# xlite-dev/LeetCUDA

Measured on AMD Instinct MI355X. Metric: achieved fp16 TFLOPS vs MI355X MFMA peak: HGEMM 8192^3; FA-2 fwd S=4096 D=128, higher is better.
Workload: dtype f16 (fp32 MFMA accumulate)

## Files before the change

### leetcuda_amd/csrc/hgemm_w4y.hip

```cpp
#pragma once
#include "hgemm_w4x.hip"

namespace lc {

struct W4yNNSrc {
  const char* ub;
  unsigned b_off[2];
  unsigned bq, bkt;
};
LC_DEVINL void w4y_nn_src_init(W4yNNSrc& s, const half_t* B, int n0, int N, int wave, int lane) {
  const int pp = lane & 15, kr = lane >> 4;
#pragma unroll
  for (int par = 0; par < 2; ++par) {
    const int pair = (pp >> 1) ^ ((kr << 1) | par);
    s.b_off[par] = (unsigned)kr * (unsigned)N * 2u + (unsigned)((pair * 2 + (pp & 1)) * 16);
  }
  s.ub = (const char*)(B + (size_t)(wave * 16) * N + n0);
  s.bq = (unsigned)N * 8u;
  s.bkt = (unsigned)N * 128u;
}

template <bool ALPHA = false>
LC_DEVINL void w4y_epilogue_b2(char* slot, half_t* C, int N, int m0, int n0, int wave, int wr, int wc, int lane, float alpha = 1.f) {
  asm volatile("" : "+v"(lane));
// ... 158 lines not shown
    const u32x4_t w4y_rb = {(uint32_t)__builtin_amdgcn_readfirstlane((uint32_t)pb),
                            (uint32_t)__builtin_amdgcn_readfirstlane((uint32_t)(pb >> 32)) & 0xffffu, 0x7fffffffu, 0x00020000u};
    const uint32_t w4y_a0 = __builtin_amdgcn_readfirstlane(lds_addr32(smem));
    const uint32_t w4y_wv = (uint32_t)wave * 1024u;
    const uint32_t w4y_blk = __builtin_amdgcn_readfirstlane((uint32_t)src.a_blk);
    const uint32_t w4y_ao0 = src.a_off[0], w4y_ao1 = src.a_off[1];
    uint32_t w4y_t, w4y_acur, w4y_anxt, w4y_b0, w4y_b1, w4y_b2, w4y_soff, w4y_t2off, w4y_tmp, w4y_swp;
    if constexpr (B_KN) {
      const uint32_t w4y_wvb = (uint32_t)wave * 4096u;
      const uint32_t w4y_bq = __builtin_amdgcn_readfirstlane(nsrc.bq), w4y_bkt = __builtin_amdgcn_readfirstlane(nsrc.bkt);
      const uint32_t w4y_bo0 = nsrc.b_off[0], w4y_bo1 = nsrc.b_off[1];
      const int ti = lane & 15, tg = lane >> 4;
      const uint32_t w4y_bk = (uint32_t)(wc * HALF_BYTES + (8 * tg + (ti >> 2)) * 256 + (ti & 3) * 8);
      const uint32_t w4y_key = (uint32_t)(((ti >> 2) << 1) | (tg & 1));
      uint32_t w4y_t2offb;
#include "hgemm_w4y_loop_nn.inc"
    } else if constexpr (SCHED == 0) {
#include "hgemm_w4y_loop0.inc"
    } else if constexpr (SCHED == 1) {
#include "hgemm_w4y_loop1.inc"
#ifdef LC_DIAG
    } else if constexpr (SCHED == 3) {
#include "hgemm_w4y_loop3.inc"
    } else if constexpr (SCHED == 4) {
#include "hgemm_w4y_loop4.inc"
    } else if constexpr (SCHED == 5) {
#include "hgemm_w4y_loop5.inc"
    } else if constexpr (SCHED == 6) {
#include "hgemm_w4y_loop2.inc"
#endif
    } else {
// ... 22 lines not shown
```

### leetcuda_amd/csrc/tu_plan.hip

```cpp
#include <stdio.h>
#include <string.h>

#include <algorithm>

#include "lc_plan.h"

namespace lc {

#define LC_KNOB(name, dflt, valid, diag) tune_t g_tune_##name{dflt};
#include "lc_knobs.inc"

Knobs read_knobs() {
  Knobs k;
#define LC_KNOB(name, dflt, valid, diag)
#define LC_KNOB_SNAP(name, dflt, valid, diag) k.name = g_tune_##name;
#include "lc_knobs.inc"
  return k;
}

namespace {
bool ok_attn_nw(int v) {
  return v == 0 || v == 512 || v == 513 || v == 514 || v == 515 || v == 517 || v == 8 || v == 4 || v == 2;
}
bool ok_01(int v) { return v == 0 || v == 1; }
// ... 263 lines not shown
  if (knob == 0 || T <= ncu || R == 0 || !(knob == 3 ? 4 * R <= 3 * ncu : knob == 4 || 2 * R <= ncu)) return t;
  t.nblk = T - R;
  if (mid_ok && knob != 2) {
    t.tmw = tile_knob == 1 ? 1 : tile_knob == 2 ? 2 : (8 * R <= ncu ? 1 : 2);
    t.ns = (t.tmw == 1 ? 8 : 4) * R <= ncu ? 3 : 2;
  }
  return t;
}

}

int plan_hgemm(const Knobs& k, int M, int N, int K, bool b_kn, int variant, bool al, HgemmPlan* out) {
  HgemmPlan p{};
  p.k = k;
  p.variant = variant;
  p.sched = b_kn ? 1 : k.w4y_sched;
  p.tail = TailSplit{-1, 0, 0, 0};
  const bool k64 = K % BK == 0, k32 = K % 32 == 0 && K >= BK;
  const bool tiles256 = (M % BM == 0) && (N % BN == 0) && k64 && al;
  const bool tiles128 = (M % BM1 == 0) && (N % BN1 == 0) && k32 && al;
  const bool edge_ok = al && K % 8 == 0 && (!b_kn || N % 8 == 0);
  const bool w4y_ok = tiles128 && M >= BM && N >= BN && w4_effective_variant(LC_HGEMM_MFMA256W4Y, b_kn, N, K) == LC_HGEMM_MFMA256W4Y;
  if (variant == LC_HGEMM_AUTO) {
    const long wg256 = (long)(M / BM) * (N / BN), rcu = rule_cus(k);
    const bool tiles64 = (M % 64 == 0) && (N % 64 == 0) && k32 && al;
    p.mid = mid_tile_auto(k, M, N, K, b_kn, true);
    if (2 * wg256 > rcu && (tiles256 || (k.hgemm_auto == LC_HGEMM_MFMA256W4Y && w4y_ok))) {
      p.fam = wg256 < rcu && p.mid.tmw > 0 && p.mid.wgs > wg256 ? HFam::MID : HFam::TILE256;
      p.variant = k.hgemm_auto;
    } else {
      p.rag = tiles128 ? RaggedPlan{0, 0, 0, 0, 0, 0, 1} : ragged_plan(k, M, N, K, al, b_kn, true);
// ... 380 lines not shown
```

### leetcuda_amd/csrc/tu_w4.hip

```cpp
#include "lc_launch.h"
#include "hgemm_w4y.hip"

namespace lc {
namespace {
template <bool B_KN, bool BUF, int DG>
int launch_w4_one(const half_t* A, const half_t* B, half_t* C, int M, int N, int K, int tiles_m, int tiles_n, int pw,
                  hipStream_t st) {
  auto kern = hgemm_w4b_kernel<B_KN, BUF, DG>;
  if (int rc = set_dyn_lds(kern, W4B_LDS)) return rc;
  hipLaunchKernelGGL(kern, dim3(tiles_m * tiles_n), dim3(256), W4B_LDS, st, A, B, C, M, N, K, tiles_m, tiles_n, pw);
  return check_launch();
}

template <bool B_KN, int Y>
int launch_w4x_one(const half_t* A, const half_t* B, half_t* C, int M, int N, int K, int tiles_m, int tiles_n, int pw,
                   int nblk_arg, hipStream_t st) {
  auto kern = [] {
    if constexpr (Y < 0) return hgemm_w4x_kernel<B_KN>;
    else return hgemm_w4y_kernel<B_KN, Y>;
  }();
  if (int rc = set_dyn_lds(kern, W4B_LDS)) return rc;
  const int nblk = nblk_arg > 0 ? nblk_arg : tiles_m * tiles_n;
  if constexpr (Y < 0) {
    hipLaunchKernelGGL(kern, dim3(nblk), dim3(256), W4B_LDS, st, A, B, C, M, N, K, tiles_m, tiles_n, pw);
// ... 23 lines not shown
#endif
  if constexpr (!B_KN) {
    if (variant == LC_HGEMM_MFMA256W4X) return launch_w4x_one<B_KN, -1>(A, B, C, M, N, K, tiles_m, tiles_n, pw, nblk, st);
    if (variant == LC_HGEMM_MFMA256W4Y) {
      if (sched == 0) return launch_w4x_one<B_KN, 0>(A, B, C, M, N, K, tiles_m, tiles_n, pw, nblk, st);
      if (sched == 1) return launch_w4x_one<B_KN, 1>(A, B, C, M, N, K, tiles_m, tiles_n, pw, nblk, st);
#ifdef LC_DIAG
      if (sched == 3) return launch_w4x_one<B_KN, 3>(A, B, C, M, N, K, tiles_m, tiles_n, pw, nblk, st);
      if (sched == 4) return launch_w4x_one<B_KN, 4>(A, B, C, M, N, K, tiles_m, tiles_n, pw, nblk, st);
      if (sched == 5) return launch_w4x_one<B_KN, 5>(A, B, C, M, N, K, tiles_m, tiles_n, pw, nblk, st);
      if (sched == 6) return launch_w4x_one<B_KN, 6>(A, B, C, M, N, K, tiles_m, tiles_n, pw, nblk, st);
#endif
      return launch_w4x_one<B_KN, 2>(A, B, C, M, N, K, tiles_m, tiles_n, pw, nblk, st);
    }
  } else {
    if (variant == LC_HGEMM_MFMA256W4Y) return launch_w4x_one<B_KN, 1>(A, B, C, M, N, K, tiles_m, tiles_n, pw, nblk, st);
  }
  if (variant == LC_HGEMM_MFMA256W4C || variant == LC_HGEMM_MFMA256W4X || variant == LC_HGEMM_MFMA256W4Y)
    return launch_w4_one<B_KN, true, 0>(A, B, C, M, N, K, tiles_m, tiles_n, pw, st);
  return launch_w4_one<B_KN, false, 0>(A, B, C, M, N, K, tiles_m, tiles_n, pw, st);
}
}

int launch_w4_family(const half_t* A, const half_t* B, half_t* C, int M, int N, int K, int variant, int sched, int stamps, int abl, bool b_kn,
                     int tiles_m, int tiles_n, int panel_w, int nblk, hipStream_t st) {
  return b_kn ? launch_w4_t<true>(A, B, C, M, N, K, variant, sched, stamps, abl, tiles_m, tiles_n, panel_w, nblk, st)
              : launch_w4_t<false>(A, B, C, M, N, K, variant, sched, stamps, abl, tiles_m, tiles_n, panel_w, nblk, st);
}
}
```

Before: 1500.

## Add paired double-buffered B-fragment loop for NN (B_KN) W4Y HGEMM path

Adds a new hand-scheduled inline-asm main loop for the B_KN (row-major B) W4Y kernel. It double-buffers the transposed B register fragments (ds_read_b64_tr_b16 into alternating v128-191 / v192-255 banks) so the next iteration's B reads interleave with the current iteration's MFMAs, and the loop is unrolled in pairs. The old NN loop stays reachable only under LC_DIAG with sched 6. It uses nearly the whole VGPR file and depends on the exact order of waitcnts and barriers, so it raises register pressure and the risk of scheduling hazards.

```diff
diff --git a/leetcuda_amd/csrc/hgemm_w4y.hip b/leetcuda_amd/csrc/hgemm_w4y.hip
--- a/leetcuda_amd/csrc/hgemm_w4y.hip
+++ b/leetcuda_amd/csrc/hgemm_w4y.hip
@@ -196,7 +196,14 @@
       const uint32_t w4y_bk = (uint32_t)(wc * HALF_BYTES + (8 * tg + (ti >> 2)) * 256 + (ti & 3) * 8);
       const uint32_t w4y_key = (uint32_t)(((ti >> 2) << 1) | (tg & 1));
       uint32_t w4y_t2offb;
+#ifdef LC_DIAG
+      if constexpr (SCHED == 6) {
 #include "hgemm_w4y_loop_nn.inc"
+      } else
+#endif
+      {
+#include "hgemm_w4y_loop_nn_pair.inc"
+      }
     } else if constexpr (SCHED == 0) {
 #include "hgemm_w4y_loop0.inc"
     } else if constexpr (SCHED == 1) {
diff --git a/leetcuda_amd/csrc/hgemm_w4y_loop_nn_pair.inc b/leetcuda_amd/csrc/hgemm_w4y_loop_nn_pair.inc
--- /dev/null
+++ b/leetcuda_amd/csrc/hgemm_w4y_loop_nn_pair.inc
@@ -0,0 +1,610 @@
+asm volatile(
+    "s_mov_b32 %[t], 0\n\t"
+    "s_mov_b32 %[acur], %[a0]\n\t"
+    "s_add_u32 %[anxt], %[a0], 0x8000\n\t"
+    "s_add_u32 %[b0], %[a0], 0x10000\n\t"
+    "s_add_u32 %[b1], %[a0], 0x18000\n\t"
+    "s_add_u32 %[b2], %[a0], 0x20000\n\t"
+    "v_xor_b32_e32 v56, 0, %[key]\n\t"
+    "v_xor_b32_e32 v57, 1, %[key]\n\t"
+    "v_xor_b32_e32 v58, 2, %[key]\n\t"
+    "v_xor_b32_e32 v59, 3, %[key]\n\t"
+    "v_xor_b32_e32 v60, 4, %[key]\n\t"
+    "v_xor_b32_e32 v61, 5, %[key]\n\t"
+    "v_xor_b32_e32 v62, 6, %[key]\n\t"
+    "v_xor_b32_e32 v63, 7, %[key]\n\t"
+    "v_lshl_add_u32 v56, v56, 5, %[bk]\n\t"
+    "v_lshl_add_u32 v57, v57, 5, %[bk]\n\t"
+    "v_lshl_add_u32 v58, v58, 5, %[bk]\n\t"
+    "v_lshl_add_u32 v59, v59, 5, %[bk]\n\t"
+    "v_lshl_add_u32 v60, v60, 5, %[bk]\n\t"
+    "v_lshl_add_u32 v61, v61, 5, %[bk]\n\t"
+    "v_lshl_add_u32 v62, v62, 5, %[bk]\n\t"
+    "v_lshl_add_u32 v63, v63, 5, %[bk]\n\t"
+    "v_add_u32_e32 v56, %[b0], v56\n\t"
+    "v_add_u32_e32 v57, %[b0], v57\n\t"
+    "v_add_u32_e32 v58, %[b0], v58\n\t"
+    "v_add_u32_e32 v59, %[b0], v59\n\t"
+    "v_add_u32_e32 v60, %[b0], v60\n\t"
+    "v_add_u32_e32 v61, %[b0], v61\n\t"
+    "v_add_u32_e32 v62, %[b0], v62\n\t"
+    "v_add_u32_e32 v63, %[b0], v63\n\t"
+    "v_add_u32_e32 v54, %[acur], %[ar0]\n\t"
+    "v_add_u32_e32 v55, %[acur], %[ar1]\n\t"
+    "ds_read_b128 v[64:67], v54 offset:0\n\t"
+    "ds_read_b128 v[96:99], v55 offset:0\n\t"
+    "ds_read_b64_tr_b16 v[128:129], v56 offset:0\n\t"
+    "ds_read_b64_tr_b16 v[130:131], v56 offset:1024\n\t"
+    "ds_read_b64_tr_b16 v[160:161], v56 offset:8192\n\t"
+    "ds_read_b64_tr_b16 v[162:163], v56 offset:9216\n\t"
+    "ds_read_b64_tr_b16 v[132:133], v57 offset:0\n\t"
+    "ds_read_b64_tr_b16 v[134:135], v57 offset:1024\n\t"
+    "ds_read_b64_tr_b16 v[164:165], v57 offset:8192\n\t"
+    "ds_read_b64_tr_b16 v[166:167], v57 offset:9216\n\t"
+    "ds_read_b64_tr_b16 v[136:137], v58 offset:0\n\t"
+    "ds_read_b64_tr_b16 v[138:139], v58 offset:1024\n\t"
+    "ds_read_b64_tr_b16 v[168:169], v58 offset:8192\n\t"
+    "ds_read_b64_tr_b16 v[170:171], v58 offset:9216\n\t"
+    "ds_read_b64_tr_b16 v[140:141], v59 offset:0\n\t"
+    "ds_read_b64_tr_b16 v[142:143], v59 offset:1024\n\t"
+    "ds_read_b64_tr_b16 v[172:173], v59 offset:8192\n\t"
+    "ds_read_b64_tr_b16 v[174:175], v59 offset:9216\n\t"
+    "ds_read_b64_tr_b16 v[144:145], v60 offset:0\n\t"
+    "ds_read_b64_tr_b16 v[146:147], v60 offset:1024\n\t"
+    "ds_read_b64_tr_b16 v[176:177], v60 offset:8192\n\t"
+    "ds_read_b64_tr_b16 v[178:179], v60 offset:9216\n\t"
+    "ds_read_b64_tr_b16 v[148:149], v61 offset:0\n\t"
+    "ds_read_b64_tr_b16 v[150:151], v61 offset:1024\n\t"
+    "ds_read_b64_tr_b16 v[180:181], v61 offset:8192\n\t"
+    "ds_read_b64_tr_b16 v[182:183], v61 offset:9216\n\t"
+    "ds_read_b64_tr_b16 v[152:153], v62 offset:0\n\t"
+    "ds_read_b64_tr_b16 v[154:155], v62 offset:1024\n\t"
+    "ds_read_b64_tr_b16 v[184:185], v62 offset:8192\n\t"
+    "ds_read_b64_tr_b16 v[186:187], v62 offset:9216\n\t"
+    "ds_read_b64_tr_b16 v[156:157], v63 offset:0\n\t"
+    "ds_read_b64_tr_b16 v[158:159], v63 offset:1024\n\t"
+    "ds_read_b64_tr_b16 v[188:189], v63 offset:8192\n\t"
+    "ds_read_b64_tr_b16 v[190:191], v63 offset:9216\n\t"
+    "s_sub_u32 %[swp], %[kt], 1\n\t"
+    "s_min_u32 %[swp], %[swp], 2\n\t"
+    "s_add_u32 %[swp], %[swp], %[stg]\n\t"
+    "s_cmp_ge_u32 %[swp], %[kt]\n\t"
+    "s_cselect_b32 %[t2off], %[kt], 0\n\t"
+    "s_sub_u32 %[swp], %[swp], %[t2off]\n\t"
+    "s_lshl_b32 %[t2off], %[swp], 7\n\t"
+    "s_mul_i32 %[t2offb], %[swp], %[bkt]\n\t"
+    ".Lw4y_loop_%=:\n\t"
+    "s_waitcnt lgkmcnt(0)\n\t"
+    "v_mfma_f32_16x16x32_f16 a[0:3], v[128:131], v[64:67], a[0:3]\n\t"
+    "v_mfma_f32_16x16x32_f16 a[0:3], v[160:163], v[96:99], a[0:3]\n\t"
+    "ds_read_b128 v[68:71], v54 offset:2048\n\t"
+    "v_mfma_f32_16x16x32_f16 a[4:7], v[132:135], v[64:67], a[4:7]\n\t"
+    "s_add_u32 %[tmp], %[b2], %[wvb]\n\t"
+    "v_mfma_f32_16x16x32_f16 a[4:7], v[164:167], v[96:99], a[4:7]\n\t"
+    "s_add_u32 m0, %[tmp], 0\n\t"
+    "s_mov_b32 %[soff], %[t2offb]\n\t"
+    "v_mfma_f32_16x16x32_f16 a[8:11], v[136:139], v[64:67], a[8:11]\n\t"
+    "buffer_load_dwordx4 %[bo0], %[rb], %[soff] offen lds\n\t"
+    "v_mfma_f32_16x16x32_f16 a[8:11], v[168:171], v[96:99], a[8:11]\n\t"
+    "ds_read_b128 v[100:103], v55 offset:2048\n\t"
+    "v_mfma_f32_16x16x32_f16 a[12:15], v[140:143], v[64:67], a[12:15]\n\t"
+    "v_mfma_f32_16x16x32_f16 a[12:15], v[172:175], v[96:99], a[12:15]\n\t"
+    "v_mfma_f32_16x16x32_f16 a[16:19], v[144:147], v[64:67], a[16:19]\n\t"
+    "v_mfma_f32_16x16x32_f16 a[16:19], v[176:179], v[96:99], a[16:19]\n\t"
+    "ds_read_b128 v[72:75], v54 offset:4096\n\t"
+    "v_mfma_f32_16x16x32_f16 a[20:23], v[148:151], v[64:67], a[20:23]\n\t"
+    "v_mfma_f32_16x16x32_f16 a[20:23], v[180:183], v[96:99], a[20:23]\n\t"
+    "s_add_u32 m0, %[tmp], 1024\n\t"
+    "s_add_u32 %[soff], %[soff], %[bq]\n\t"
+    "v_mfma_f32_16x16x32_f16 a[24:27], v[152:155], v[64:67], a[24:27]\n\t"
+    "buffer_load_dwordx4 %[bo0], %[rb], %[soff] offen lds\n\t"
+    "v_mfma_f32_16x16x32_f16 a[24:27], v[184:187], v[96:99], a[24:27]\n\t"
+    "ds_read_b128 v[104:107], v55 offset:4096\n\t"
+    "v_mfma_f32_16x16x32_f16 a[28:31], v[156:159], v[64:67], a[28:31]\n\t"
+    "v_mfma_f32_16x16x32_f16 a[28:31], v[188:191], v[96:99], a[28:31]\n\t"
+    "s_waitcnt lgkmcnt(2)\n\t"
+    "v_mfma_f32_16x16x32_f16 a[32:35], v[128:131], v[68:71], a[32:35]\n\t"
+    "v_mfma_f32_16x16x32_f16 a[32:35], v[160:163], v[100:103], a[32:35]\n\t"
+    "ds_read_b128 v[76:79], v54 offset:6144\n\t"
+    "v_mfma_f32_16x16x32_f16 a[36:39], v[132:135], v[68:71], a[36:39]\n\t"
+    "v_mfma_f32_16x16x32_f16 a[36:39], v[164:167], v[100:103], a[36:39]\n\t"
+    "s_add_u32 m0, %[tmp], 2048\n\t"
+    "s_add_u32 %[soff], %[soff], %[bq]\n\t"
+    "v_mfma_f32_16x16x32_f16 a[40:43], v[136:139], v[68:71], a[40:43]\n\t"
+    "buffer_load_dwordx4 %[bo1], %[rb], %[soff] offen lds\n\t"
+    "v_mfma_f32_16x16x32_f16 a[40:43], v[168:171], v[100:103], a[40:43]\n\t"
+    "ds_read_b128 v[108:111], v55 offset:6144\n\t"
+    "v_mfma_f32_16x16x32_f16 a[44:47], v[140:143], v[68:71], a[44:47]\n\t"
+    "v_mfma_f32_16x16x32_f16 a[44:47], v[172:175], v[100:103], a[44:47]\n\t"
+    "v_mfma_f32_16x16x32_f16 a[48:51], v[144:147], v[68:71], a[48:51]\n\t"
+    "v_mfma_f32_16x16x32_f16 a[48:51], v[176:179], v[100:103], a[48:51]\n\t"
+    "ds_read_b128 v[80:83], v54 offset:8192\n\t"
+    "v_mfma_f32_16x16x32_f16 a[52:55], v[148:151], v[68:71], a[52:55]\n\t"
+    "v_mfma_f32_16x16x32_f16 a[52:55], v[180:183], v[100:103], a[52:55]\n\t"
+    "s_add_u32 m0, %[tmp], 3072\n\t"
+    "s_add_u32 %[soff], %[soff], %[bq]\n\t"
+    "v_mfma_f32_16x16x32_f16 a[56:59], v[152:155], v[68:71], a[56:59]\n\t"
+    "buffer_load_dwordx4 %[bo1], %[rb], %[soff] offen lds\n\t"
+    "v_mfma_f32_16x16x32_f16 a[56:59], v[184:187], v[100:103], a[56:59]\n\t"
+    "ds_read_b128 v[112:115], v55 offset:8192\n\t"
+    "v_mfma_f32_16x16x32_f16 a[60:63], v[156:159], v[68:71], a[60:63]\n\t"
+    "v_mfma_f32_16x16x32_f16 a[60:63], v[188:191], v[100:103], a[60:63]\n\t"
+    "s_waitcnt lgkmcnt(4)\n\t"
+    "v_mfma_f32_16x16x32_f16 a[64:67], v[128:131], v[72:75], a[64:67]\n\t"
+    "v_mfma_f32_16x16x32_f16 a[64:67], v[160:163], v[104:107], a[64:67]\n\t"
+    "ds_read_b128 v[84:87], v54 offset:10240\n\t"
+    "v_mfma_f32_16x16x32_f16 a[68:71], v[132:135], v[72:75], a[68:71]\n\t"
+    "v_mfma_f32_16x16x32_f16 a[68:71], v[164:167], v[104:107], a[68:71]\n\t"
+    "s_add_u32 m0, %[tmp], 16384\n\t"
+    "s_add_u32 %[soff], %[t2offb], 256\n\t"
+    "v_mfma_f32_16x16x32_f16 a[72:75], v[136:139], v[72:75], a[72:75]\n\t"
+    "buffer_load_dwordx4 %[bo0], %[rb], %[soff] offen lds\n\t"
+    "v_mfma_f32_16x16x32_f16 a[72:75], v[168:171], v[104:107], a[72:75]\n\t"
+    "ds_read_b128 v[116:119], v55 offset:10240\n\t"
+    "v_mfma_f32_16x16x32_f16 a[76:79], v[140:143], v[72:75], a[76:79]\n\t"
+    "v_mfma_f32_16x16x32_f16 a[76:79], v[172:175], v[104:107], a[76:79]\n\t"
+    "v_mfma_f32_16x16x32_f16 a[80:83], v[144:147], v[72:75], a[80:83]\n\t"
+    "v_mfma_f32_16x16x32_f16 a[80:83], v[176:179], v[104:107], a[80:83]\n\t"
+    "ds_read_b128 v[88:91], v54 offset:12288\n\t"
+    "v_mfma_f32_16x16x32_f16 a[84:87], v[148:151], v[72:75], a[84:87]\n\t"
+    "v_mfma_f32_16x16x32_f16 a[84:87], v[180:183], v[104:107], a[84:87]\n\t"
+    "s_add_u32 m0, %[tmp], 17408\n\t"
+    "s_add_u32 %[soff], %[soff], %[bq]\n\t"
+    "v_mfma_f32_16x16x32_f16 a[88:91], v[152:155], v[72:75], a[88:91]\n\t"
+    "buffer_load_dwordx4 %[bo0], %[rb], %[soff] offen lds\n\t"
+    "v_mfma_f32_16x16x32_f16 a[88:91], v[184:187], v[104:107], a[88:91]\n\t"
+    "ds_read_b128 v[120:123], v55 offset:12288\n\t"
+    "v_mfma_f32_16x16x32_f16 a[92:95], v[156:159], v[72:75], a[92:95]\n\t"
+    "v_mfma_f32_16x16x32_f16 a[92:95], v[188:191], v[104:107], a[92:95]\n\t"
+    "s_waitcnt lgkmcnt(6)\n\t"
+    "v_mfma_f32_16x16x32_f16 a[96:99], v[128:131], v[76:79], a[96:99]\n\t"
+    "v_mfma_f32_16x16x32_f16 a[96:99], v[160:163], v[108:111], a[96:99]\n\t"
+    "ds_read_b128 v[92:95], v54 offset:14336\n\t"
+    "v_mfma_f32_16x16x32_f16 a[100:103], v[132:135], v[76:79], a[100:103]\n\t"
+    "v_mfma_f32_16x16x32_f16 a[100:103], v[164:167], v[108:111], a[100:103]\n\t"
+    "s_add_u32 m0, %[tmp], 18432\n\t"
+    "s_add_u32 %[soff], %[soff], %[bq]\n\t"
+    "v_mfma_f32_16x16x32_f16 a[104:107], v[136:139], v[76:79], a[104:107]\n\t"
+    "buffer_load_dwordx4 %[bo1], %[rb], %[soff] offen lds\n\t"
+    "v_mfma_f32_16x16x32_f16 a[104:107], v[168:171], v[108:111], a[104:107]\n\t"
+    "ds_read_b128 v[124:127], v55 offset:14336\n\t"
+    "v_mfma_f32_16x16x32_f16 a[108:111], v[140:143], v[76:79], a[108:111]\n\t"
+    "v_mfma_f32_16x16x32_f16 a[108:111], v[172:175], v[108:111], a[108:111]\n\t"
+    "v_mfma_f32_16x16x32_f16 a[112:115], v[144:147], v[76:79], a[112:115]\n\t"
+    "v_mfma_f32_16x16x32_f16 a[112:115], v[176:179], v[108:111], a[112:115]\n\t"
+    "v_mfma_f32_16x16x32_f16 a[116:119], v[148:151], v[76:79], a[116:119]\n\t"
+    "v_mfma_f32_16x16x32_f16 a[116:119], v[180:183], v[108:111], a[116:119]\n\t"
+    "s_add_u32 m0, %[tmp], 19456\n\t"
+    "s_add_u32 %[soff], %[soff], %[bq]\n\t"
+    "v_mfma_f32_16x16x32_f16 a[120:123], v[152:155], v[76:79], a[120:123]\n\t"
+    "buffer_load_dwordx4 %[bo1], %[rb], %[soff] offen lds\n\t"
+    "v_mfma_f32_16x16x32_f16 a[120:123], v[184:187], v[108:111], a[120:123]\n\t"
+    "v_mfma_f32_16x16x32_f16 a[124:127], v[156:159], v[76:79], a[124:127]\n\t"
+    "v_mfma_f32_16x16x32_f16 a[124:127], v[188:191], v[108:111], a[124:127]\n\t"
+    "s_waitcnt vmcnt(8) lgkmcnt(0)\n\t"
+    "v_mfma_f32_16x16x32_f16 a[128:131], v[128:131], v[80:83], a[128:131]\n\t"
+    "s_barrier\n\t"
+    "v_add_u32_e32 v54, %[anxt], %[ar0]\n\t"
+    "s_add_u32 %[tmp], %[acur], %[wv]\n\t"
+    "s_sub_u32 %[swp], %[b1], %[b0]\n\t"
+    "v_mfma_f32_16x16x32_f16 a[128:131], v[160:163], v[112:115], a[128:131]\n\t"
+    "v_add_u32_e32 v55, %[anxt], %[ar1]\n\t"
+    "v_add_u32_e32 v56, %[swp], v56\n\t"
+    "v_add_u32_e32 v57, %[swp], v57\n\t"
+    "v_mfma_f32_16x16x32_f16 a[132:135], v[132:135], v[80:83], a[132:135]\n\t"
+    "s_add_u32 m0, %[tmp], 0\n\t"
+    "s_mov_b32 %[soff], %[t2off]\n\t"
+    "v_add_u32_e32 v58, %[swp], v58\n\t"
+    "v_add_u32_e32 v59, %[swp], v59\n\t"
+    "v_mfma_f32_16x16x32_f16 a[132:135], v[164:167], v[112:115], a[132:135]\n\t"
+    "buffer_load_dwordx4 %[ao0], %[ra], %[soff] offen lds\n\t"
+    "v_add_u32_e32 v60, %[swp], v60\n\t"
+    "v_add_u32_e32 v61, %[swp], v61\n\t"
+    "v_mfma_f32_16x16x32_f16 a[136:139], v[136:139], v[80:83], a[136:139]\n\t"
+    "v_add_u32_e32 v62, %[swp], v62\n\t"
+    "ds_read_b128 v[64:67], v54 offset:0\n\t"
+    "v_mfma_f32_16x16x32_f16 a[136:139], v[168:171], v[112:115], a[136:139]\n\t"
+    "v_add_u32_e32 v63, %[swp], v63\n\t"
+    "ds_read_b128 v[96:99], v55 offset:0\n\t"
+    "v_mfma_f32_16x16x32_f16 a[140:143], v[140:143], v[80:83], a[140:143]\n\t"
+    "ds_read_b64_tr_b16 v[192:193], v56 offset:0\n\t"
+    "v_mfma_f32_16x16x32_f16 a[140:143], v[172:175], v[112:115], a[140:143]\n\t"
+    "ds_read_b64_tr_b16 v[194:195], v56 offset:1024\n\t"
+    "v_mfma_f32_16x16x32_f16 a[144:147], v[144:147], v[80:83], a[144:147]\n\t"
+    "s_mov_b32 %[swp], %[b0]\n\t"
+    "s_mov_b32 %[b0], %[b1]\n\t"
+    "s_mov_b32 %[b1], %[b2]\n\t"
+    "s_mov_b32 %[b2], %[swp]\n\t"
+    "s_mov_b32 %[swp], %[acur]\n\t"
+    "s_mov_b32 %[acur], %[anxt]\n\t"
+    "v_mfma_f32_16x16x32_f16 a[144:147], v[176:179], v[112:115], a[144:147]\n\t"
+    "s_add_u32 m0, %[tmp], 4096\n\t"
+    "s_add_u32 %[soff], %[soff], %[blk]\n\t"
+    "v_mfma_f32_16x16x32_f16 a[148:151], v[148:151], v[80:83], a[148:151]\n\t"
+    "buffer_load_dwordx4 %[ao1], %[ra], %[soff] offen lds\n\t"
+    "v_mfma_f32_16x16x32_f16 a[148:151], v[180:183], v[112:115], a[148:151]\n\t"
+    "ds_read_b64_tr_b16 v[224:225], v56 offset:8192\n\t"
+    "v_mfma_f32_16x16x32_f16 a[152:155], v[152:155], v[80:83], a[152:155]\n\t"
+    "ds_read_b64_tr_b16 v[226:227], v56 offset:9216\n\t"
+    "v_mfma_f32_16x16x32_f16 a[152:155], v[184:187], v[112:115], a[152:155]\n\t"
+    "ds_read_b64_tr_b16 v[196:197], v57 offset:0\n\t"
+    "v_mfma_f32_16x16x32_f16 a[156:159], v[156:159], v[80:83], a[156:159]\n\t"
+    "s_mov_b32 %[anxt], %[swp]\n\t"
+    "v_mfma_f32_16x16x32_f16 a[156:159], v[188:191], v[112:115], a[156:159]\n\t"
+    "ds_read_b64_tr_b16 v[198:199], v57 offset:1024\n\t"
+    "v_mfma_f32_16x16x32_f16 a[160:163], v[128:131], v[84:87], a[160:163]\n\t"
+    "s_add_u32 m0, %[tmp], 8192\n\t"
+    "s_add_u32 %[soff], %[soff], %[blk]\n\t"
+    "v_mfma_f32_16x16x32_f16 a[160:163], v[160:163], v[116:119], a[160:163]\n\t"
+    "buffer_load_dwordx4 %[ao0], %[ra], %[soff] offen lds\n\t"
+    "v_mfma_f32_16x16x32_f16 a[164:167], v[132:135], v[84:87], a[164:167]\n\t"
+    "ds_read_b64_tr_b16 v[228:229], v57 offset:8192\n\t"
+    "v_mfma_f32_16x16x32_f16 a[164:167], v[164:167], v[116:119], a[164:167]\n\t"
+    "ds_read_b64_tr_b16 v[230:231], v57 offset:9216\n\t"
+    "v_mfma_f32_16x16x32_f16 a[168:171], v[136:139], v[84:87], a[168:171]\n\t"
+    "ds_read_b64_tr_b16 v[200:201], v58 offset:0\n\t"
+    "v_mfma_f32_16x16x32_f16 a[168:171], v[168:171], v[116:119], a[168:171]\n\t"
+    "s_add_u32 %[swp], %[t], 3\n\t"
+    "v_mfma_f32_16x16x32_f16 a[172:175], v[140:143], v[84:87], a[172:175]\n\t"
+    "ds_read_b64_tr_b16 v[202:203], v58 offset:1024\n\t"
+    "v_mfma_f32_16x16x32_f16 a[172:175], v[172:175], v[116:119], a[172:175]\n\t"
+    "s_add_u32 m0, %[tmp], 12288\n\t"
+    "s_add_u32 %[soff], %[soff], %[blk]\n\t"
+    "v_mfma_f32_16x16x32_f16 a[176:179], v[144:147], v[84:87], a[176:179]\n\t"
+    "buffer_load_dwordx4 %[ao1], %[ra], %[soff] offen lds\n\t"
+    "v_mfma_f32_16x16x32_f16 a[176:179], v[176:179], v[116:119], a[176:179]\n\t"
+    "ds_read_b64_tr_b16 v[232:233], v58 offset:8192\n\t"
+    "v_mfma_f32_16x16x32_f16 a[180:183], v[148:151], v[84:87], a[180:183]\n\t"
+    "ds_read_b64_tr_b16 v[234:235], v58 offset:9216\n\t"
+    "v_mfma_f32_16x16x32_f16 a[180:183], v[180:183], v[116:119], a[180:183]\n\t"
+    "s_sub_u32 %[t2off], %[kt], 1\n\t"
+    "v_mfma_f32_16x16x32_f16 a[184:187], v[152:155], v[84:87], a[184:187]\n\t"
+    "ds_read_b64_tr_b16 v[204:205], v59 offset:0\n\t"
+    "v_mfma_f32_16x16x32_f16 a[184:187], v[184:187], v[116:119], a[184:187]\n\t"
+    "ds_read_b64_tr_b16 v[206:207], v59 offset:1024\n\t"
+    "v_mfma_f32_16x16x32_f16 a[188:191], v[156:159], v[84:87], a[188:191]\n\t"
+    "s_add_u32 m0, %[tmp], 16384\n\t"
+    "s_add_u32 %[soff], %[soff], %[blk]\n\t"
+    "v_mfma_f32_16x16x32_f16 a[188:191], v[188:191], v[116:119], a[188:191]\n\t"
+    "buffer_load_dwordx4 %[ao0], %[ra], %[soff] offen lds\n\t"
+    "v_mfma_f32_16x16x32_f16 a[192:195], v[128:131], v[88:91], a[192:195]\n\t"
+    "ds_read_b64_tr_b16 v[236:237], v59 offset:8192\n\t"
+    "v_mfma_f32_16x16x32_f16 a[192:195], v[160:163], v[120:123], a[192:195]\n\t"
+    "s_min_u32 %[swp], %[swp], %[t2off]\n\t"
+    "v_mfma_f32_16x16x32_f16 a[196:199], v[132:135], v[88:91], a[196:199]\n\t"
+    "ds_read_b64_tr_b16 v[238:239], v59 offset:9216\n\t"
+    "v_mfma_f32_16x16x32_f16 a[196:199], v[164:167], v[120:123], a[196:199]\n\t"
+    "ds_read_b64_tr_b16 v[208:209], v60 offset:0\n\t"
+    "v_mfma_f32_16x16x32_f16 a[200:203], v[136:139], v[88:91], a[200:203]\n\t"
+    "ds_read_b64_tr_b16 v[210:211], v60 offset:1024\n\t"
+    "v_mfma_f32_16x16x32_f16 a[200:203], v[168:171], v[120:123], a[200:203]\n\t"
+    "s_add_u32 m0, %[tmp], 20480\n\t"
+    "s_add_u32 %[soff], %[soff], %[blk]\n\t"
+    "v_mfma_f32_16x16x32_f16 a[204:207], v[140:143], v[88:91], a[204:207]\n\t"
+    "buffer_load_dwordx4 %[ao1], %[ra], %[soff] offen lds\n\t"
+    "v_mfma_f32_16x16x32_f16 a[204:207], v[172:175], v[120:123], a[204:207]\n\t"
+    "ds_read_b64_tr_b16 v[240:241], v60 offset:8192\n\t"
+    "v_mfma_f32_16x16x32_f16 a[208:211], v[144:147], v[88:91], a[208:211]\n\t"
+    "s_add_u32 %[swp], %[swp], %[stg]\n\t"
+    "v_mfma_f32_16x16x32_f16 a[208:211], v[176:179], v[120:123], a[208:211]\n\t"
+    "ds_read_b64_tr_b16 v[242:243], v60 offset:9216\n\t"
+    "v_mfma_f32_16x16x32_f16 a[212:215], v[148:151], v[88:91], a[212:215]\n\t"
+    "ds_read_b64_tr_b16 v[212:213], v61 offset:0\n\t"
+    "v_mfma_f32_16x16x32_f16 a[212:215], v[180:183], v[120:123], a[212:215]\n\t"
+    "ds_read_b64_tr_b16 v[214:215], v61 offset:1024\n\t"
+    "v_mfma_f32_16x16x32_f16 a[216:219], v[152:155], v[88:91], a[216:219]\n\t"
+    "s_add_u32 m0, %[tmp], 24576\n\t"
+    "s_add_u32 %[soff], %[soff], %[blk]\n\t"
+    "v_mfma_f32_16x16x32_f16 a[216:219], v[184:187], v[120:123], a[216:219]\n\t"
+    "buffer_load_dwordx4 %[ao0], %[ra], %[soff] offen lds\n\t"
+    "v_mfma_f32_16x16x32_f16 a[220:223], v[156:159], v[88:91], a[220:223]\n\t"
+    "s_cmp_ge_u32 %[swp], %[kt]\n\t"
+    "s_cselect_b32 %[t2off], %[kt], 0\n\t"
+    "v_mfma_f32_16x16x32_f16 a[220:223], v[188:191], v[120:123], a[220:223]\n\t"
+    "ds_read_b64_tr_b16 v[244:245], v61 offset:8192\n\t"
+    "v_mfma_f32_16x16x32_f16 a[224:227], v[128:131], v[92:95], a[224:227]\n\t"
+    "ds_read_b64_tr_b16 v[246:247], v61 offset:9216\n\t"
+    "v_mfma_f32_16x16x32_f16 a[224:227], v[160:163], v[124:127], a[224:227]\n\t"
+    "ds_read_b64_tr_b16 v[216:217], v62 offset:0\n\t"
+    "v_mfma_f32_16x16x32_f16 a[228:231], v[132:135], v[92:95], a[228:231]\n\t"
+    "ds_read_b64_tr_b16 v[218:219], v62 offset:1024\n\t"
+    "v_mfma_f32_16x16x32_f16 a[228:231], v[164:167], v[124:127], a[228:231]\n\t"
+    "s_add_u32 m0, %[tmp], 28672\n\t"
+    "s_add_u32 %[soff], %[soff], %[blk]\n\t"
+    "v_mfma_f32_16x16x32_f16 a[232:235], v[136:139], v[92:95], a[232:235]\n\t"
+    "buffer_load_dwordx4 %[ao1], %[ra], %[soff] offen lds\n\t"
+    "v_mfma_f32_16x16x32_f16 a[232:235], v[168:171], v[124:127], a[232:235]\n\t"
+    "s_sub_u32 %[swp], %[swp], %[t2off]\n\t"
+    "v_mfma_f32_16x16x32_f16 a[236:239], v[140:143], v[92:95], a[236:239]\n\t"
+    "ds_read_b64_tr_b16 v[248:249], v62 offset:8192\n\t"
+    "v_mfma_f32_16x16x32_f16 a[236:239], v[172:175], v[124:127], a[236:239]\n\t"
+    "ds_read_b64_tr_b16 v[250:251], v62 offset:9216\n\t"
+    "v_mfma_f32_16x16x32_f16 a[240:243], v[144:147], v[92:95], a[240:243]\n\t"
+    "ds_read_b64_tr_b16 v[220:221], v63 offset:0\n\t"
+    "v_mfma_f32_16x16x32_f16 a[240:243], v[176:179], v[124:127], a[240:243]\n\t"
+    "s_lshl_b32 %[t2off], %[swp], 7\n\t"
+    "v_mfma_f32_16x16x32_f16 a[244:247], v[148:151], v[92:95], a[244:247]\n\t"
+    "ds_read_b64_tr_b16 v[222:223], v63 offset:1024\n\t"
+    "v_mfma_f32_16x16x32_f16 a[244:247], v[180:183], v[124:127], a[244:247]\n\t"
+    "ds_read_b64_tr_b16 v[252:253], v63 offset:8192\n\t"
+    "v_mfma_f32_16x16x32_f16 a[248:251], v[152:155], v[92:95], a[248:251]\n\t"
+    "ds_read_b64_tr_b16 v[254:255], v63 offset:9216\n\t"
+    "v_mfma_f32_16x16x32_f16 a[248:251], v[184:187], v[124:127], a[248:251]\n\t"
+    "s_mul_i32 %[t2offb], %[swp], %[bkt]\n\t"
+    "v_mfma_f32_16x16x32_f16 a[252:255], v[156:159], v[92:95], a[252:255]\n\t"
+    "s_add_u32 %[t], %[t], 1\n\t"
+    "s_cmp_lt_u32 %[t], %[kt]\n\t"
+    "v_mfma_f32_16x16x32_f16 a[252:255], v[188:191], v[124:127], a[252:255]\n\t"
+    "s_cbranch_scc0 .Lw4y_exit_%=\n\t"
+    "s_waitcnt lgkmcnt(0)\n\t"
+    "v_mfma_f32_16x16x32_f16 a[0:3], v[192:195], v[64:67], a[0:3]\n\t"
+    "v_mfma_f32_16x16x32_f16 a[0:3], v[224:227], v[96:99], a[0:3]\n\t"
+    "ds_read_b128 v[68:71], v54 offset:2048\n\t"
+    "v_mfma_f32_16x16x32_f16 a[4:7], v[196:199], v[64:67], a[4:7]\n\t"
+    "s_add_u32 %[tmp], %[b2], %[wvb]\n\t"
+    "v_mfma_f32_16x16x32_f16 a[4:7], v[228:231], v[96:99], a[4:7]\n\t"
+    "s_add_u32 m0, %[tmp], 0\n\t"
+    "s_mov_b32 %[soff], %[t2offb]\n\t"
+    "v_mfma_f32_16x16x32_f16 a[8:11], v[200:203], v[64:67], a[8:11]\n\t"
+    "buffer_load_dwordx4 %[bo0], %[rb], %[soff] offen lds\n\t"
+    "v_mfma_f32_16x16x32_f16 a[8:11], v[232:235], v[96:99], a[8:11]\n\t"
+    "ds_read_b128 v[100:103], v55 offset:2048\n\t"
+    "v_mfma_f32_16x16x32_f16 a[12:15], v[204:207], v[64:67], a[12:15]\n\t"
+    "v_mfma_f32_16x16x32_f16 a[12:15], v[236:239], v[96:99], a[12:15]\n\t"
+    "v_mfma_f32_16x16x32_f16 a[16:19], v[208:211], v[64:67], a[16:19]\n\t"
+    "v_mfma_f32_16x16x32_f16 a[16:19], v[240:243], v[96:99], a[16:19]\n\t"
+    "ds_read_b128 v[72:75], v54 offset:4096\n\t"
+    "v_mfma_f32_16x16x32_f16 a[20:23], v[212:215], v[64:67], a[20:23]\n\t"
+    "v_mfma_f32_16x16x32_f16 a[20:23], v[244:247], v[96:99], a[20:23]\n\t"
+    "s_add_u32 m0, %[tmp], 1024\n\t"
+    "s_add_u32 %[soff], %[soff], %[bq]\n\t"
+    "v_mfma_f32_16x16x32_f16 a[24:27], v[216:219], v[64:67], a[24:27]\n\t"
+    "buffer_load_dwordx4 %[bo0], %[rb], %[soff] offen lds\n\t"
+    "v_mfma_f32_16x16x32_f16 a[24:27], v[248:251], v[96:99], a[24:27]\n\t"
+    "ds_read_b128 v[104:107], v55 offset:4096\n\t"
+    "v_mfma_f32_16x16x32_f16 a[28:31], v[220:223], v[64:67], a[28:31]\n\t"
+    "v_mfma_f32_16x16x32_f16 a[28:31], v[252:255], v[96:99], a[28:31]\n\t"
+    "s_waitcnt lgkmcnt(2)\n\t"
+    "v_mfma_f32_16x16x32_f16 a[32:35], v[192:195], v[68:71], a[32:35]\n\t"
+    "v_mfma_f32_16x16x32_f16 a[32:35], v[224:227], v[100:103], a[32:35]\n\t"
+    "ds_read_b128 v[76:79], v54 offset:6144\n\t"
+    "v_mfma_f32_16x16x32_f16 a[36:39], v[196:199], v[68:71], a[36:39]\n\t"
+    "v_mfma_f32_16x16x32_f16 a[36:39], v[228:231], v[100:103], a[36:39]\n\t"
+    "s_add_u32 m0, %[tmp], 2048\n\t"
+    "s_add_u32 %[soff], %[soff], %[bq]\n\t"
+    "v_mfma_f32_16x16x32_f16 a[40:43], v[200:203], v[68:71], a[40:43]\n\t"
+    "buffer_load_dwordx4 %[bo1], %[rb], %[soff] offen lds\n\t"
+    "v_mfma_f32_16x16x32_f16 a[40:43], v[232:235], v[100:103], a[40:43]\n\t"
+    "ds_read_b128 v[108:111], v55 offset:6144\n\t"
+    "v_mfma_f32_16x16x32_f16 a[44:47], v[204:207], v[68:71], a[44:47]\n\t"
+    "v_mfma_f32_16x16x32_f16 a[44:47], v[236:239], v[100:103], a[44:47]\n\t"
+    "v_mfma_f32_16x16x32_f16 a[48:51], v[208:211], v[68:71], a[48:51]\n\t"
+    "v_mfma_f32_16x16x32_f16 a[48:51], v[240:243], v[100:103], a[48:51]\n\t"
+    "ds_read_b128 v[80:83], v54 offset:8192\n\t"
+    "v_mfma_f32_16x16x32_f16 a[52:55], v[212:215], v[68:71], a[52:55]\n\t"
+    "v_mfma_f32_16x16x32_f16 a[52:55], v[244:247], v[100:103], a[52:55]\n\t"
+    "s_add_u32 m0, %[tmp], 3072\n\t"
+    "s_add_u32 %[soff], %[soff], %[bq]\n\t"
+    "v_mfma_f32_16x16x32_f16 a[56:59], v[216:219], v[68:71], a[56:59]\n\t"
+    "buffer_load_dwordx4 %[bo1], %[rb], %[soff] offen lds\n\t"
+    "v_mfma_f32_16x16x32_f16 a[56:59], v[248:251], v[100:103], a[56:59]\n\t"
+    "ds_read_b128 v[112:115], v55 offset:8192\n\t"
+    "v_mfma_f32_16x16x32_f16 a[60:63], v[220:223], v[68:71], a[60:63]\n\t"
+    "v_mfma_f32_16x16x32_f16 a[60:63], v[252:255], v[100:103], a[60:63]\n\t"
+    "s_waitcnt lgkmcnt(4)\n\t"
+    "v_mfma_f32_16x16x32_f16 a[64:67], v[192:195], v[72:75], a[64:67]\n\t"
+    "v_mfma_f32_16x16x32_f16 a[64:67], v[224:227], v[104:107], a[64:67]\n\t"
+    "ds_read_b128 v[84:87], v54 offset:10240\n\t"
+    "v_mfma_f32_16x16x32_f16 a[68:71], v[196:199], v[72:75], a[68:71]\n\t"
+    "v_mfma_f32_16x16x32_f16 a[68:71], v[228:231], v[104:107], a[68:71]\n\t"
+    "s_add_u32 m0, %[tmp], 16384\n\t"
+    "s_add_u32 %[soff], %[t2offb], 256\n\t"
+    "v_mfma_f32_16x16x32_f16 a[72:75], v[200:203], v[72:75], a[72:75]\n\t"
+    "buffer_load_dwordx4 %[bo0], %[rb], %[soff] offen lds\n\t"
+    "v_mfma_f32_16x16x32_f16 a[72:75], v[232:235], v[104:107], a[72:75]\n\t"
+    "ds_read_b128 v[116:119], v55 offset:10240\n\t"
+    "v_mfma_f32_16x16x32_f16 a[76:79], v[204:207], v[72:75], a[76:79]\n\t"
+    "v_mfma_f32_16x16x32_f16 a[76:79], v[236:239], v[104:107], a[76:79]\n\t"
+    "v_mfma_f32_16x16x32_f16 a[80:83], v[208:211], v[72:75], a[80:83]\n\t"
+    "v_mfma_f32_16x16x32_f16 a[80:83], v[240:243], v[104:107], a[80:83]\n\t"
+    "ds_read_b128 v[88:91], v54 offset:12288\n\t"
+    "v_mfma_f32_16x16x32_f16 a[84:87], v[212:215], v[72:75], a[84:87]\n\t"
+    "v_mfma_f32_16x16x32_f16 a[84:87], v[244:247], v[104:107], a[84:87]\n\t"
+    "s_add_u32 m0, %[tmp], 17408\n\t"
+    "s_add_u32 %[soff], %[soff], %[bq]\n\t"
+    "v_mfma_f32_16x16x32_f16 a[88:91], v[216:219], v[72:75], a[88:91]\n\t"
+    "buffer_load_dwordx4 %[bo0], %[rb], %[soff] offen lds\n\t"
+    "v_mfma_f32_16x16x32_f16 a[88:91], v[248:251], v[104:107], a[88:91]\n\t"
+    "ds_read_b128 v[120:123], v55 offset:12288\n\t"
+    "v_mfma_f32_16x16x32_f16 a[92:95], v[220:223], v[72:75], a[92:95]\n\t"
+    "v_mfma_f32_16x16x32_f16 a[92:95], v[252:255], v[104:107], a[92:95]\n\t"
+    "s_waitcnt lgkmcnt(6)\n\t"
+    "v_mfma_f32_16x16x32_f16 a[96:99], v[192:195], v[76:79], a[96:99]\n\t"
+    "v_mfma_f32_16x16x32_f16 a[96:99], v[224:227], v[108:111], a[96:99]\n\t"
+    "ds_read_b128 v[92:95], v54 offset:14336\n\t"
+    "v_mfma_f32_16x16x32_f16 a[100:103], v[196:199], v[76:79], a[100:103]\n\t"
+    "v_mfma_f32_16x16x32_f16 a[100:103], v[228:231], v[108:111], a[100:103]\n\t"
+    "s_add_u32 m0, %[tmp], 18432\n\t"
+    "s_add_u32 %[soff], %[soff], %[bq]\n\t"
+    "v_mfma_f32_16x16x32_f16 a[104:107], v[200:203], v[76:79], a[104:107]\n\t"
+    "buffer_load_dwordx4 %[bo1], %[rb], %[soff] offen lds\n\t"
+    "v_mfma_f32_16x16x32_f16 a[104:107], v[232:235], v[108:111], a[104:107]\n\t"
+    "ds_read_b128 v[124:127], v55 offset:14336\n\t"
+    "v_mfma_f32_16x16x32_f16 a[108:111], v[204:207], v[76:79], a[108:111]\n\t"
+    "v_mfma_f32_16x16x32_f16 a[108:111], v[236:239], v[108:111], a[108:111]\n\t"
+    "v_mfma_f32_16x16x32_f16 a[112:115], v[208:211], v[76:79], a[112:115]\n\t"
+    "v_mfma_f32_16x16x32_f16 a[112:115], v[240:243], v[108:111], a[112:115]\n\t"
+    "v_mfma_f32_16x16x32_f16 a[116:119], v[212:215], v[76:79], a[116:119]\n\t"
+    "v_mfma_f32_16x16x32_f16 a[116:119], v[244:247], v[108:111], a[116:119]\n\t"
+    "s_add_u32 m0, %[tmp], 19456\n\t"
+    "s_add_u32 %[soff], %[soff], %[bq]\n\t"
+    "v_mfma_f32_16x16x32_f16 a[120:123], v[216:219], v[76:79], a[120:123]\n\t"
+    "buffer_load_dwordx4 %[bo1], %[rb], %[soff] offen lds\n\t"
+    "v_mfma_f32_16x16x32_f16 a[120:123], v[248:251], v[108:111], a[120:123]\n\t"
+    "v_mfma_f32_16x16x32_f16 a[124:127], v[220:223], v[76:79], a[124:127]\n\t"
+    "v_mfma_f32_16x16x32_f16 a[124:127], v[252:255], v[108:111], a[124:127]\n\t"
+    "s_waitcnt vmcnt(8) lgkmcnt(0)\n\t"
+    "v_mfma_f32_16x16x32_f16 a[128:131], v[192:195], v[80:83], a[128:131]\n\t"
+    "s_barrier\n\t"
+    "v_add_u32_e32 v54, %[anxt], %[ar0]\n\t"
+    "s_add_u32 %[tmp], %[acur], %[wv]\n\t"
+    "s_sub_u32 %[swp], %[b1], %[b0]\n\t"
+    "v_mfma_f32_16x16x32_f16 a[128:131], v[224:227], v[112:115], a[128:131]\n\t"
+    "v_add_u32_e32 v55, %[anxt], %[ar1]\n\t"
+    "v_add_u32_e32 v56, %[swp], v56\n\t"
+    "v_add_u32_e32 v57, %[swp], v57\n\t"
+    "v_mfma_f32_16x16x32_f16 a[132:135], v[196:199], v[80:83], a[132:135]\n\t"
+    "s_add_u32 m0, %[tmp], 0\n\t"
+    "s_mov_b32 %[soff], %[t2off]\n\t"
+    "v_add_u32_e32 v58, %[swp], v58\n\t"
+    "v_add_u32_e32 v59, %[swp], v59\n\t"
+    "v_mfma_f32_16x16x32_f16 a[132:135], v[228:231], v[112:115], a[132:135]\n\t"
+    "buffer_load_dwordx4 %[ao0], %[ra], %[soff] offen lds\n\t"
+    "v_add_u32_e32 v60, %[swp], v60\n\t"
+    "v_add_u32_e32 v61, %[swp], v61\n\t"
+    "v_mfma_f32_16x16x32_f16 a[136:139], v[200:203], v[80:83], a[136:139]\n\t"
+    "v_add_u32_e32 v62, %[swp], v62\n\t"
+    "ds_read_b128 v[64:67], v54 offset:0\n\t"
+    "v_mfma_f32_16x16x32_f16 a[136:139], v[232:235], v[112:115], a[136:139]\n\t"
+    "v_add_u32_e32 v63, %[swp], v63\n\t"
+    "ds_read_b128 v[96:99], v55 offset:0\n\t"
+    "v_mfma_f32_16x16x32_f16 a[140:143], v[204:207], v[80:83], a[140:143]\n\t"
+    "ds_read_b64_tr_b16 v[128:129], v56 offset:0\n\t"
+    "v_mfma_f32_16x16x32_f16 a[140:143], v[236:239], v[112:115], a[140:143]\n\t"
+    "ds_read_b64_tr_b16 v[130:131], v56 offset:1024\n\t"
+    "v_mfma_f32_16x16x32_f16 a[144:147], v[208:211], v[80:83], a[144:147]\n\t"
+    "s_mov_b32 %[swp], %[b0]\n\t"
+    "s_mov_b32 %[b0], %[b1]\n\t"
+    "s_mov_b32 %[b1], %[b2]\n\t"
+    "s_mov_b32 %[b2], %[swp]\n\t"
+    "s_mov_b32 %[swp], %[acur]\n\t"
+    "s_mov_b32 %[acur], %[anxt]\n\t"
+    "v_mfma_f32_16x16x32_f16 a[144:147], v[240:243], v[112:115], a[144:147]\n\t"
+    "s_add_u32 m0, %[tmp], 4096\n\t"
+    "s_add_u32 %[soff], %[soff], %[blk]\n\t"
+    "v_mfma_f32_16x16x32_f16 a[148:151], v[212:215], v[80:83], a[148:151]\n\t"
+    "buffer_load_dwordx4 %[ao1], %[ra], %[soff] offen lds\n\t"
+    "v_mfma_f32_16x16x32_f16 a[148:151], v[244:247], v[112:115], a[148:151]\n\t"
+    "ds_read_b64_tr_b16 v[160:161], v56 offset:8192\n\t"
+    "v_mfma_f32_16x16x32_f16 a[152:155], v[216:219], v[80:83], a[152:155]\n\t"
+    "ds_read_b64_tr_b16 v[162:163], v56 offset:9216\n\t"
+    "v_mfma_f32_16x16x32_f16 a[152:155], v[248:251], v[112:115], a[152:155]\n\t"
+    "ds_read_b64_tr_b16 v[132:133], v57 offset:0\n\t"
+    "v_mfma_f32_16x16x32_f16 a[156:159], v[220:223], v[80:83], a[156:159]\n\t"
+    "s_mov_b32 %[anxt], %[swp]\n\t"
+    "v_mfma_f32_16x16x32_f16 a[156:159], v[252:255], v[112:115], a[156:159]\n\t"
+    "ds_read_b64_tr_b16 v[134:135], v57 offset:1024\n\t"
+    "v_mfma_f32_16x16x32_f16 a[160:163], v[192:195], v[84:87], a[160:163]\n\t"
+    "s_add_u32 m0, %[tmp], 8192\n\t"
+    "s_add_u32 %[soff], %[soff], %[blk]\n\t"
+    "v_mfma_f32_16x16x32_f16 a[160:163], v[224:227], v[116:119], a[160:163]\n\t"
+    "buffer_load_dwordx4 %[ao0], %[ra], %[soff] offen lds\n\t"
+    "v_mfma_f32_16x16x32_f16 a[164:167], v[196:199], v[84:87], a[164:167]\n\t"
+    "ds_read_b64_tr_b16 v[164:165], v57 offset:8192\n\t"
+    "v_mfma_f32_16x16x32_f16 a[164:167], v[228:231], v[116:119], a[164:167]\n\t"
+    "ds_read_b64_tr_b16 v[166:167], v57 offset:9216\n\t"
+    "v_mfma_f32_16x16x32_f16 a[168:171], v[200:203], v[84:87], a[168:171]\n\t"
+    "ds_read_b64_tr_b16 v[136:137], v58 offset:0\n\t"
+    "v_mfma_f32_16x16x32_f16 a[168:171], v[232:235], v[116:119], a[168:171]\n\t"
+    "s_add_u32 %[swp], %[t], 3\n\t"
+    "v_mfma_f32_16x16x32_f16 a[172:175], v[204:207], v[84:87], a[172:175]\n\t"
+    "ds_read_b64_tr_b16 v[138:139], v58 offset:1024\n\t"
+    "v_mfma_f32_16x16x32_f16 a[172:175], v[236:239], v[116:119], a[172:175]\n\t"
+    "s_add_u32 m0, %[tmp], 12288\n\t"
+    "s_add_u32 %[soff], %[soff], %[blk]\n\t"
+    "v_mfma_f32_16x16x32_f16 a[176:179], v[208:211], v[84:87], a[176:179]\n\t"
+    "buffer_load_dwordx4 %[ao1], %[ra], %[soff] offen lds\n\t"
+    "v_mfma_f32_16x16x32_f16 a[176:179], v[240:243], v[116:119], a[176:179]\n\t"
+    "ds_read_b64_tr_b16 v[168:169], v58 offset:8192\n\t"
+    "v_mfma_f32_16x16x32_f16 a[180:183], v[212:215], v[84:87], a[180:183]\n\t"
+    "ds_read_b64_tr_b16 v[170:171], v58 offset:9216\n\t"
+    "v_mfma_f32_16x16x32_f16 a[180:183], v[244:247], v[116:119], a[180:183]\n\t"
+    "s_sub_u32 %[t2off], %[kt], 1\n\t"
+    "v_mfma_f32_16x16x32_f16 a[184:187], v[216:219], v[84:87], a[184:187]\n\t"
+    "ds_read_b64_tr_b16 v[140:141], v59 offset:0\n\t"
+    "v_mfma_f32_16x16x32_f16 a[184:187], v[248:251], v[116:119], a[184:187]\n\t"
+    "ds_read_b64_tr_b16 v[142:143], v59 offset:1024\n\t"
+    "v_mfma_f32_16x16x32_f16 a[188:191], v[220:223], v[84:87], a[188:191]\n\t"
+    "s_add_u32 m0, %[tmp], 16384\n\t"
+    "s_add_u32 %[soff], %[soff], %[blk]\n\t"
+    "v_mfma_f32_16x16x32_f16 a[188:191], v[252:255], v[116:119], a[188:191]\n\t"
+    "buffer_load_dwordx4 %[ao0], %[ra], %[soff] offen lds\n\t"
+    "v_mfma_f32_16x16x32_f16 a[192:195], v[192:195], v[88:91], a[192:195]\n\t"
+    "ds_read_b64_tr_b16 v[172:173], v59 offset:8192\n\t"
+    "v_mfma_f32_16x16x32_f16 a[192:195], v[224:227], v[120:123], a[192:195]\n\t"
+    "s_min_u32 %[swp], %[swp], %[t2off]\n\t"
+    "v_mfma_f32_16x16x32_f16 a[196:199], v[196:199], v[88:91], a[196:199]\n\t"
+    "ds_read_b64_tr_b16 v[174:175], v59 offset:9216\n\t"
+    "v_mfma_f32_16x16x32_f16 a[196:199], v[228:231], v[120:123], a[196:199]\n\t"
+    "ds_read_b64_tr_b16 v[144:145], v60 offset:0\n\t"
+    "v_mfma_f32_16x16x32_f16 a[200:203], v[200:203], v[88:91], a[200:203]\n\t"
+    "ds_read_b64_tr_b16 v[146:147], v60 offset:1024\n\t"
+    "v_mfma_f32_16x16x32_f16 a[200:203], v[232:235], v[120:123], a[200:203]\n\t"
+    "s_add_u32 m0, %[tmp], 20480\n\t"
+    "s_add_u32 %[soff], %[soff], %[blk]\n\t"
+    "v_mfma_f32_16x16x32_f16 a[204:207], v[204:207], v[88:91], a[204:207]\n\t"
+    "buffer_load_dwordx4 %[ao1], %[ra], %[soff] offen lds\n\t"
+    "v_mfma_f32_16x16x32_f16 a[204:207], v[236:239], v[120:123], a[204:207]\n\t"
+    "ds_read_b64_tr_b16 v[176:177], v60 offset:8192\n\t"
+    "v_mfma_f32_16x16x32_f16 a[208:211], v[208:211], v[88:91], a[208:211]\n\t"
+    "s_add_u32 %[swp], %[swp], %[stg]\n\t"
+    "v_mfma_f32_16x16x32_f16 a[208:211], v[240:243], v[120:123], a[208:211]\n\t"
+    "ds_read_b64_tr_b16 v[178:179], v60 offset:9216\n\t"
+    "v_mfma_f32_16x16x32_f16 a[212:215], v[212:215], v[88:91], a[212:215]\n\t"
+    "ds_read_b64_tr_b16 v[148:149], v61 offset:0\n\t"
+    "v_mfma_f32_16x16x32_f16 a[212:215], v[244:247], v[120:123], a[212:215]\n\t"
+    "ds_read_b64_tr_b16 v[150:151], v61 offset:1024\n\t"
+    "v_mfma_f32_16x16x32_f16 a[216:219], v[216:219], v[88:91], a[216:219]\n\t"
+    "s_add_u32 m0, %[tmp], 24576\n\t"
+    "s_add_u32 %[soff], %[soff], %[blk]\n\t"
+    "v_mfma_f32_16x16x32_f16 a[216:219], v[248:251], v[120:123], a[216:219]\n\t"
+    "buffer_load_dwordx4 %[ao0], %[ra], %[soff] offen lds\n\t"
+    "v_mfma_f32_16x16x32_f16 a[220:223], v[220:223], v[88:91], a[220:223]\n\t"
+    "s_cmp_ge_u32 %[swp], %[kt]\n\t"
+    "s_cselect_b32 %[t2off], %[kt], 0\n\t"
+    "v_mfma_f32_16x16x32_f16 a[220:223], v[252:255], v[120:123], a[220:223]\n\t"
+    "ds_read_b64_tr_b16 v[180:181], v61 offset:8192\n\t"
+    "v_mfma_f32_16x16x32_f16 a[224:227], v[192:195], v[92:95], a[224:227]\n\t"
+    "ds_read_b64_tr_b16 v[182:183], v61 offset:9216\n\t"
+    "v_mfma_f32_16x16x32_f16 a[224:227], v[224:227], v[124:127], a[224:227]\n\t"
+    "ds_read_b64_tr_b16 v[152:153], v62 offset:0\n\t"
+    "v_mfma_f32_16x16x32_f16 a[228:231], v[196:199], v[92:95], a[228:231]\n\t"
+    "ds_read_b64_tr_b16 v[154:155], v62 offset:1024\n\t"
+    "v_mfma_f32_16x16x32_f16 a[228:231], v[228:231], v[124:127], a[228:231]\n\t"
+    "s_add_u32 m0, %[tmp], 28672\n\t"
+    "s_add_u32 %[soff], %[soff], %[blk]\n\t"
+    "v_mfma_f32_16x16x32_f16 a[232:235], v[200:203], v[92:95], a[232:235]\n\t"
+    "buffer_load_dwordx4 %[ao1], %[ra], %[soff] offen lds\n\t"
+    "v_mfma_f32_16x16x32_f16 a[232:235], v[232:235], v[124:127], a[232:235]\n\t"
+    "s_sub_u32 %[swp], %[swp], %[t2off]\n\t"
+    "v_mfma_f32_16x16x32_f16 a[236:239], v[204:207], v[92:95], a[236:239]\n\t"
+    "ds_read_b64_tr_b16 v[184:185], v62 offset:8192\n\t"
+    "v_mfma_f32_16x16x32_f16 a[236:239], v[236:239], v[124:127], a[236:239]\n\t"
+    "ds_read_b64_tr_b16 v[186:187], v62 offset:9216\n\t"
+    "v_mfma_f32_16x16x32_f16 a[240:243], v[208:211], v[92:95], a[240:243]\n\t"
+    "ds_read_b64_tr_b16 v[156:157], v63 offset:0\n\t"
+    "v_mfma_f32_16x16x32_f16 a[240:243], v[240:243], v[124:127], a[240:243]\n\t"
+    "s_lshl_b32 %[t2off], %[swp], 7\n\t"
+    "v_mfma_f32_16x16x32_f16 a[244:247], v[212:215], v[92:95], a[244:247]\n\t"
+    "ds_read_b64_tr_b16 v[158:159], v63 offset:1024\n\t"
+    "v_mfma_f32_16x16x32_f16 a[244:247], v[244:247], v[124:127], a[244:247]\n\t"
+    "ds_read_b64_tr_b16 v[188:189], v63 offset:8192\n\t"
+    "v_mfma_f32_16x16x32_f16 a[248:251], v[216:219], v[92:95], a[248:251]\n\t"
+    "ds_read_b64_tr_b16 v[190:191], v63 offset:9216\n\t"
+    "v_mfma_f32_16x16x32_f16 a[248:251], v[248:251], v[124:127], a[248:251]\n\t"
+    "s_mul_i32 %[t2offb], %[swp], %[bkt]\n\t"
+    "v_mfma_f32_16x16x32_f16 a[252:255], v[220:223], v[92:95], a[252:255]\n\t"
+    "s_add_u32 %[t], %[t], 1\n\t"
+    "s_cmp_lt_u32 %[t], %[kt]\n\t"
+    "v_mfma_f32_16x16x32_f16 a[252:255], v[252:255], v[124:127], a[252:255]\n\t"
+    "s_cbranch_scc1 .Lw4y_loop_%=\n\t"
+    ".Lw4y_exit_%=:\n\t"
+    "s_waitcnt vmcnt(0) lgkmcnt(0)\n\t"
+    : [t] "=&s"(w4y_t), [acur] "=&s"(w4y_acur), [anxt] "=&s"(w4y_anxt), [b0] "=&s"(w4y_b0), [b1] "=&s"(w4y_b1),
+      [b2] "=&s"(w4y_b2), [soff] "=&s"(w4y_soff), [t2off] "=&s"(w4y_t2off), [t2offb] "=&s"(w4y_t2offb),
+      [tmp] "=&s"(w4y_tmp), [swp] "=&s"(w4y_swp)
+    : [kt] "s"(KT), [stg] "s"(w4y_stg), [a0] "s"(w4y_a0), [wv] "s"(w4y_wv), [wvb] "s"(w4y_wvb), [blk] "s"(w4y_blk), [bq] "s"(w4y_bq),
+      [bkt] "s"(w4y_bkt), [ra] "s"(w4y_ra), [rb] "s"(w4y_rb), [ao0] "v"(w4y_ao0), [ao1] "v"(w4y_ao1),
+      [bo0] "v"(w4y_bo0), [bo1] "v"(w4y_bo1), [ar0] "v"(fr.a_ad[0]), [ar1] "v"(fr.a_ad[1]), [bk] "v"(w4y_bk),
+      [key] "v"(w4y_key)
+    : "memory", "scc", "v54", "v55", "v56", "v57", "v58", "v59", "v60", "v61", "v62", "v63", "v64", "v65", "v66", "v67", "v68", "v69", "v70", "v71", "v72", "v73", "v74", "v75", "v76", "v77", "v78", "v79", "v80", "v81", "v82", "v83", "v84", "v85", "v86", "v87", "v88", "v89", "v90", "v91", "v92", "v93", "v94", "v95", "v96", "v97", "v98", "v99", "v100", "v101", "v102", "v103", "v104", "v105", "v106", "v107", "v108", "v109", "v110", "v111", "v112", "v113", "v114", "v115", "v116", "v117", "v118", "v119", "v120", "v121", "v122", "v123", "v124", "v125", "v126", "v127", "v128", "v129", "v130", "v131", "v132", "v133", "v134", "v135", "v136", "v137", "v138", "v139", "v140", "v141", "v142", "v143", "v144", "v145", "v146", "v147", "v148", "v149", "v150", "v151", "v152", "v153", "v154", "v155", "v156", "v157", "v158", "v159", "v160", "v161", "v162", "v163", "v164", "v165", "v166", "v167", "v168", "v169", "v170", "v171", "v172", "v173", "v174", "v175", "v176", "v177", "v178", "v179", "v180", "v181", "v182", "v183", "v184", "v185", "v186", "v187", "v188", "v189", "v190", "v191", "v192", "v193", "v194", "v195", "v196", "v197", "v198", "v199", "v200", "v201", "v202", "v203", "v204", "v205", "v206", "v207", "v208", "v209", "v210", "v211", "v212", "v213", "v214", "v215", "v216", "v217", "v218", "v219", "v220", "v221", "v222", "v223", "v224", "v225", "v226", "v227", "v228", "v229", "v230", "v231", "v232", "v233", "v234", "v235", "v236", "v237", "v238", "v239", "v240", "v241", "v242", "v243", "v244", "v245", "v246", "v247", "v248", "v249", "v250", "v251", "v252", "v253", "v254", "v255", LC_AGPR_ALL);
diff --git a/leetcuda_amd/csrc/tu_plan.hip b/leetcuda_amd/csrc/tu_plan.hip
--- a/leetcuda_amd/csrc/tu_plan.hip
+++ b/leetcuda_amd/csrc/tu_plan.hip
@@ -301,7 +301,11 @@
   HgemmPlan p{};
   p.k = k;
   p.variant = variant;
+#ifdef LC_DIAG
+  p.sched = b_kn ? (k.w4y_sched == 6 ? 6 : 1) : k.w4y_sched;
+#else
   p.sched = b_kn ? 1 : k.w4y_sched;
+#endif
   p.tail = TailSplit{-1, 0, 0, 0};
   const bool k64 = K % BK == 0, k32 = K % 32 == 0 && K >= BK;
   const bool tiles256 = (M % BM == 0) && (N % BN == 0) && k64 && al;
diff --git a/leetcuda_amd/csrc/tu_w4.hip b/leetcuda_amd/csrc/tu_w4.hip
--- a/leetcuda_amd/csrc/tu_w4.hip
+++ b/leetcuda_amd/csrc/tu_w4.hip
@@ -61,6 +61,9 @@
       return launch_w4x_one<B_KN, 2>(A, B, C, M, N, K, tiles_m, tiles_n, pw, nblk, st);
     }
   } else {
+#ifdef LC_DIAG
+    if (variant == LC_HGEMM_MFMA256W4Y && sched == 6) return launch_w4x_one<B_KN, 6>(A, B, C, M, N, K, tiles_m, tiles_n, pw, nblk, st);
+#endif
     if (variant == LC_HGEMM_MFMA256W4Y) return launch_w4x_one<B_KN, 1>(A, B, C, M, N, K, tiles_m, tiles_n, pw, nblk, st);
   }
   if (variant == LC_HGEMM_MFMA256W4C || variant == LC_HGEMM_MFMA256W4X || variant == LC_HGEMM_MFMA256W4Y)
```

Result: no change. 1499 (-0.0%).
